# zhao-zilong/Fed-TGAN

Measured on AMD Instinct MI355X. Metric: sec_per_epoch, lower is better.
Workload: dtype bf16; 1 GPU; model=Fed-TGAN CTGAN (G 256x256 residual+BN, D 256x256 pack10, WGAN-GP slerp), global_batch=500, parallelism=fed1, rows_per_client=40000, n_sample=40000, steps_per_epoch=80, backend=hip, data_plane=none

## Files before the change

### csrc/bindings.cpp

```cpp
#include <ATen/ATen.h>
#include <c10/hip/HIPStream.h>
#include <torch/library.h>

#include <cstring>
#include <utility>
#include <string>
#include <vector>

#include "comm/rccl_comm.h"
#include "host/csv_writer.h"
#include "kernels/launch.h"

using at::Tensor;
using c10::optional;

namespace {

hipStream_t cur_stream() { return c10::hip::getCurrentHIPStream().stream(); }

void check_f32_2d(const Tensor& t, const char* name) {
  TORCH_CHECK(t.is_cuda(), name, " must be a GPU tensor");
  TORCH_CHECK(t.scalar_type() == at::kFloat, name, " must be float32");
  TORCH_CHECK(t.dim() == 2, name, " must be 2-D");
  TORCH_CHECK(t.size(1) <= 1 || t.stride(1) == 1, name, " must have unit column stride");
// ... 2016 lines not shown
bool is_checked() { return true; }
#else
bool is_checked() { return false; }
#endif

std::string py_float(double x) { return fedtgan::format_py_float(x); }

int64_t set_tuning(const std::string& key, int64_t value) {
  if (key == "colown_dbg") {
    TORCH_CHECK(value >= 0 && value <= 7, "colown_dbg: bit mask 0..7");
    const int64_t prev = fedtgan::g_colown_dbg;
    fedtgan::g_colown_dbg = (int)value;
    return prev;
  }
  if (key == "bn_cols") {
    TORCH_CHECK(value == 4 || value == 8 || value == 16, "bn_cols must be 4, 8 or 16");
    const int64_t prev = fedtgan::g_bn_cols;
    fedtgan::g_bn_cols = (int)value;
    return prev;
  }
  if (key == "decode_rows") {
    TORCH_CHECK(value >= 0 && value <= 2, "decode_rows: 0 per cell, 1 per row, 2 per row over Philox quads");
    const int prev = fedtgan::g_decode_rows;
    fedtgan::g_decode_rows = (int)value;
    return prev;
  }
  if (key == "chain_pre") {
    TORCH_CHECK(value >= 0 && value <= 2, "chain_pre: 0, 1 or 2");
    const int prev = fedtgan::g_chain_pre;
    fedtgan::g_chain_pre = (int)value;
    return prev;
  }
  if (key == "chain_rows") {
    TORCH_CHECK(value == 1 || value == 2, "chain_rows: 1 or 2");
    const int prev = fedtgan::g_chain_rows;
    fedtgan::g_chain_rows = (int)value;
    return prev;
  }
  if (key == "chain_coalesced") {
    const int prev = fedtgan::g_chain_coalesced;
    fedtgan::g_chain_coalesced = value ? 1 : 0;
    return prev;
  }
  if (key == "gp_threads") {
    TORCH_CHECK(value == 256 || value == 1024, "gp_threads: 256 or 1024");
    const int prev = fedtgan::g_gp_threads;
    fedtgan::g_gp_threads = (int)value;
    return prev;
  }
  if (key == "bn_threads") {
    TORCH_CHECK(value == 512 || value == 1024, "bn_threads: 512 or 1024");
    const int prev = fedtgan::g_bn_threads;
    fedtgan::g_bn_threads = (int)value;
    return prev;
  }
  if (key == "act_rowreg_narrow") {
    TORCH_CHECK(value >= 0 && value <= 2, "act_rowreg_narrow: 0, 1 or 2");
    const int prev = fedtgan::g_act_rowreg_narrow;
    fedtgan::g_act_rowreg_narrow = (int)value;
    return prev;
  }
  if (key == "gp_split") {
    const int prev = fedtgan::g_gp_split;
    fedtgan::g_gp_split = value ? 1 : 0;
    return prev;
  }
  if (key == "act_row_mode") {
    TORCH_CHECK(value >= 0 && value <= 2, "act_row_mode: 0 per-wave, 1 row (LDS image), 2 row (registers; forward)");
    const int prev = fedtgan::g_act_row_mode;
    fedtgan::g_act_row_mode = (int)value;
    return prev;
  }
  if (key == "xcd_clients") {
    TORCH_CHECK(value == 0 || value == 1, "xcd_clients: 0 or 1");
    const int64_t prev = fedtgan::g_xcd_clients;
    fedtgan::g_xcd_clients = (int)value;
    return prev;
  }
  if (key == "adam_store") {
    TORCH_CHECK(value == 0 || value == 2 || value == 16, "adam_store: 0 plain, 2 nt, 16 sc1");
    const int64_t prev = fedtgan::g_adam_store;
    fedtgan::g_adam_store = (int)value;
    return prev;
  }
  if (key == "adam_u_min") {
    TORCH_CHECK(value >= 0, "adam_u_min: >= 0");
    const int64_t prev = fedtgan::g_adam_u_min;
    fedtgan::g_adam_u_min = value;
    return prev;
  }
  if (key == "bnb_first") {
    const int64_t prev = fedtgan::g_bnb_first;
    fedtgan::g_bnb_first = value ? 1 : 0;
    return prev;
  }
  if (key == "bnb_cols") {
    TORCH_CHECK(value == 4 || value == 8, "bnb_cols: 4 or 8");
    const int64_t prev = fedtgan::g_bnb_cols;
    fedtgan::g_bnb_cols = (int)value;
    return prev;
  }
  if (key == "vgm_split") {
    TORCH_CHECK(value >= 0 && value <= 64, "vgm_split: 0..64");
    const int64_t prev = fedtgan::g_vgm_split;
    fedtgan::g_vgm_split = (int)value;
    return prev;
// ... 329 lines not shown
```

### csrc/kernels/ctgan_ops.hip

```cpp
#include <algorithm>
#include <stdexcept>
#include <string>

#include "common.h"
#include "launch.h"
#include "adam_cs.h"

namespace fedtgan {

int g_xcd_clients = 1;
ClientBatch& client_batch() {
  static thread_local ClientBatch cb{1, 0, 0, nullptr, 0};
  return cb;
}

void check_slab(const void* p, const char* what) {
  const ClientBatch& cb = client_batch();
  if (cb.k <= 1 || p == nullptr) return;
  const char* c = static_cast<const char*>(p);
  if (c < cb.base || c >= cb.base + cb.stride)
    throw std::runtime_error(std::string("batched launch: ") + what +
                             " is not in client 0's arena slab (every buffer of a batched step must be)");
}

// ... 754 lines not shown
#pragma unroll
    for (int u = 0; u < TU; ++u) {
      const int j = min(j0 + u * NTH + tid, sl.cols - 1);
      ra[u] = a[j];
      fb[u] = y[j];
    }
#pragma unroll
    for (int u = 0; u < TU; ++u) {
      const int j = j0 + u * NTH + tid;
      if (j < sl.cols) o[j] = wa * ra[u] + wb * fb[u];
    }
  }
}

template <int NW, bool BT_ = false>
__global__ __launch_bounds__(NW * 64) void activate_rowblk_kernel(const float* __restrict__ logits, int ldl,
                                                                  float* __restrict__ out, int ldo, int rows,
                                                                  SpanTables sp, float inv_tau, uint64_t seed,
                                                                  const uint64_t* ctr, uint32_t stream_id,
                                                                  SlerpFuse sl, ClientBatch cb) {
  const BIdx bi_ = batch_bidx<BT_>(cb.xcd);
  extern __shared__ float act_smem[];
  if (bi_.z) {
    const int64_t co = (int64_t)bi_.z * cb.stride;
    logits = cptr(logits, co);
    out = cptr(out, co);
    ctr = cptr(ctr, co);
    client_off(sp, co);
    client_off(sl, co);
    seed += (uint64_t)bi_.z * cb.seed_step;
  }
  constexpr int NTH = NW * 64;
  const int tid = threadIdx.x, lane = tid & 63, wv = tid >> 6;
  const int r = bi_.x;
  const int D = sp.dim, S = sp.n_span;
  const float* x = logits + (size_t)r * ldl;
  const int* einfo = sp.packed;
  const int* kind = einfo + D;
  const int* start = kind + S;
  const int* width = start + S;
  float* vs = act_smem;
  float* smax = vs + D;
  float* ssum = smax + S;
  float* red = ssum + S;
  float* y = out + (size_t)r * ldo;
  const bool do_sl = sl.real != nullptr && r < sl.rows;
  const float* a = do_sl ? sl.real + (size_t)r * sl.ld : x;
  const int j = wv * 64 + lane;
  const bool in = j < D;
  const int jc = min(j, D - 1);
  float xv = x[jc];
  const int ic = einfo[jc];
  const float ar = a[jc];
  const uint64_t step = ctr ? *ctr : 0ull;
  if (in) {
    RngArgs rng{seed, ctr, stream_id};
    const uint4 u4 = rng4(rng, step, ((uint64_t)r << 20) + (uint64_t)(wv >> 2) * 64u + (uint64_t)lane);
    const int q = wv & 3;
    const uint32_t u = q == 0 ? u4.x : q == 1 ? u4.y : q == 2 ? u4.z : u4.w;
    if (!(ic & EI_SOFTMAX)) {
      xv = tanhf(xv);
      y[j] = xv;
    } else {
      xv = (xv + gumbel(u)) * inv_tau;
      vs[j] = xv;
    }
  }
  __syncthreads();
  for (int s2 = tid; s2 < S; s2 += NTH) {
    if (kind[s2] == 0) continue;
    const int st = start[s2], w = width[s2];
    const float* v = vs + st;
    float m = -INFINITY;
    int i = 0;
    for (; i + 4 <= w; i += 4) m = fmaxf(fmaxf(m, fmaxf(v[i], v[i + 1])), fmaxf(v[i + 2], v[i + 3]));
    for (; i < w; ++i) m = fmaxf(m, v[i]);
    float e0 = 0.f, e1 = 0.f;
    i = 0;
    for (; i + 2 <= w; i += 2) {
      e0 += __expf(v[i] - m);
      e1 += __expf(v[i + 1] - m);
    }
    if (i < w) e0 += __expf(v[i] - m);
    smax[s2] = m;
    ssum[s2] = 1.f / (e0 + e1);
  }
  __syncthreads();
  if (in && (ic & EI_SOFTMAX)) {
    const int s2 = ic & (EI_SOFTMAX - 1);
    xv = __expf(xv - smax[s2]) * ssum[s2];
    y[j] = xv;
  }
  if (!do_sl) return;
  float saa = 0.f, sbb = 0.f, sab = 0.f;
  if (in) {
    saa = ar * ar;
    sbb = xv * xv;
    sab = ar * xv;
  }
  constexpr int TU = 2;
  float ra[TU], fb[TU];
#pragma unroll
  for (int u = 0; u < TU; ++u) {
    const int jt = min(D + u * NTH + tid, sl.cols - 1);
    ra[u] = a[jt];
    fb[u] = y[jt];
  }
#pragma unroll
  for (int u = 0; u < TU; ++u)
    if (D + u * NTH + tid < sl.cols) {
      saa += ra[u] * ra[u];
      sbb += fb[u] * fb[u];
      sab += ra[u] * fb[u];
    }
  for (int jt = D + TU * NTH + tid; jt < sl.cols; jt += NTH) {
    const float ra2 = a[jt], fb2 = y[jt];
    saa += ra2 * ra2;
    sbb += fb2 * fb2;
    sab += ra2 * fb2;
  }
  const float3 tot = block_sum3<NW>(saa, sbb, sab, red);
  RngArgs srng{seed, ctr, sl.stream};
  const float alpha = u01(rng4(srng, step, (uint64_t)r).x);
  float wa, wb;
  slerp_weights(tot.x, tot.y, tot.z, alpha, wa, wb);
  float* o = sl.out + (size_t)r * sl.ld;
  if (in) o[j] = wa * ar + wb * xv;
#pragma unroll
  for (int u = 0; u < TU; ++u) {
    const int jt = D + u * NTH + tid;
    if (jt < sl.cols) o[jt] = wa * ra[u] + wb * fb[u];
  }
  for (int jt = D + TU * NTH + tid; jt < sl.cols; jt += NTH) o[jt] = wa * a[jt] + wb * y[jt];
}

template <bool BT_ = false>
__global__ __launch_bounds__(ROW_WAVES * 64) void act_bwd_ce_row_kernel(const float* __restrict__ dact, int ldd,
                                                                        const float* __restrict__ act, int lda,
                                                                        const float* __restrict__ logits, int ldl,
                                                                        SpanTables sp, const int* __restrict__ col,
                                                                        const int* __restrict__ opt,
                                                                        float* __restrict__ dl, int ldg, int rows,
                                                                        float inv_tau, float* loss, int loss_per_row,
                                                                        ClientBatch cb) {
  const BIdx bi_ = batch_bidx<BT_>(cb.xcd);
  extern __shared__ float act_smem[];
  if (bi_.z) {
    const int64_t co = (int64_t)bi_.z * cb.stride;
    dact = cptr(dact, co);
    act = cptr(act, co);
    logits = cptr(logits, co);
    col = cptr(col, co);
    opt = cptr(opt, co);
    dl = cptr(dl, co);
    loss = cptr(loss, co);
    client_off(sp, co);
  }
  const int tid = threadIdx.x, lane = tid & 63, wv = tid >> 6;
  const int r = bi_.x;
  const int D = sp.dim, S = sp.n_span;
  const float* g = dact + (size_t)r * ldd;
  const float* y = act + (size_t)r * lda;
  const float* x = logits + (size_t)r * ldl;
  const int cr = col[r];
  const int orow = opt[r];
  const ActSmem t = act_stage_tables(sp, act_smem);
  float* xs = t.rows;
  float* stat = xs + D;
  int* cspan = reinterpret_cast<int*>(stat + S);
  float* lse_sh = stat + S + 1;
  float* d = dl + (size_t)r * ldg;
  for (int s2 = tid; s2 < S; s2 += blockDim.x) stat[s2] = 0.f;
  if (tid == 0) *cspan = -1;
  __syncthreads();
  for (int s2 = tid; s2 < S; s2 += blockDim.x)
    if (t.kind[s2] != 0 && t.cidx[s2] == cr) *cspan = s2;
// ... 837 lines not shown
  const float* uw = jb.dot_w ? jb.dot_w : jb.w;
  float s = 0.f, s2 = 0.f;
#pragma unroll 8
  for (int r = grp; r < jb.rows; r += CS_GROUPS) {
    const float a = jb.a[(size_t)r * jb.lda + cc];
    s += (jb.w ? jb.w[r] : 1.f) * a;
    if (jb.dot_w) s2 += jb.dot_w[r] * a;
  }
  part[0][grp][threadIdx.x % CS_COLS] = s;
  part[1][grp][threadIdx.x % CS_COLS] = s2;
  __syncthreads();
  if (grp == 0) {
    float t = 0.f, t2 = 0.f;
    for (int i = 0; i < CS_GROUPS; ++i) {
      t += part[0][i][threadIdx.x];
      t2 += part[1][i][threadIdx.x];
    }
    if (c < jb.cols && jb.out) jb.out[c] = t;
    if (jb.dot_v) {
      float d = c < jb.cols ? (jb.dot_w ? t2 : t) * jb.dot_v[c] : 0.f;
      if (bi_.x == 0 && jb.dot_e) {
        float ws = 0.f;
        for (int r = threadIdx.x; r < jb.rows; r += 64) ws += uw ? uw[r] : 1.f;
        d += wave_sum(ws) * (threadIdx.x == 0 ? jb.dot_e[0] : 0.f);
      }
      d = wave_sum(d);
      if (threadIdx.x == 0) atomicAdd(jb.dot_out, d);
    }
  }
}

void launch_colsum(const ColsumJob* jobs, int n_jobs, hipStream_t stream) {
  ColsumBatch bt{};
  int maxc = 0;
  n_jobs = std::min(n_jobs, 8);
  for (int i = 0; i < n_jobs; ++i) {
    bt.jobs[i] = jobs[i];
    maxc = std::max(maxc, jobs[i].cols);
  }
  bt.n_jobs = n_jobs;
  if (n_jobs == 0 || maxc == 0) return;
  const ClientBatch cb = client_batch();
  if (cb.k > 1)
    for (int i = 0; i < n_jobs; ++i)
      check_slabs("colsum job", bt.jobs[i].a, bt.jobs[i].out, bt.jobs[i].w, bt.jobs[i].dot_v, bt.jobs[i].dot_e,
                  bt.jobs[i].dot_out, bt.jobs[i].dot_w);
  hipLaunchKernelGGL((client_batch().xcd ? colsum_kernel<true> : colsum_kernel<false>), dim3((maxc + CS_COLS - 1) / CS_COLS, n_jobs, cb.k), dim3(CS_COLS * CS_GROUPS), 0,
                     stream, bt, cb);
}

constexpr int BN_THREADS = 512, BN_WAVES = BN_THREADS / 64;
int g_bn_cols = 8;
int g_bn_threads = 512;
static int bn_cols_for_launch() { return g_bn_cols; }

constexpr int BN_MAXG = 2;

template <int COLS, int NV, int NTH = BN_THREADS>
__device__ __forceinline__ void bn_colsum(float (&v)[NV], float* sh) {
  constexpr int NWV = NTH / 64;
  const int lane = threadIdx.x & 63, wv = threadIdx.x >> 6, lc = threadIdx.x % COLS;
#pragma unroll
  for (int k = 0; k < NV; ++k) {
#pragma unroll
    for (int o = COLS; o < 64; o <<= 1) v[k] += __shfl_xor(v[k], o, 64);
    if (lane < COLS) sh[(k * NWV + wv) * COLS + lc] = v[k];
  }
  __syncthreads();
#pragma unroll
  for (int k = 0; k < NV; ++k) {
    float t = 0.f;
#pragma unroll
    for (int w = 0; w < NWV; ++w) t += sh[(k * NWV + w) * COLS + lc];
    v[k] = t;
  }
  __syncthreads();
}

struct BnStat {
  float mu, var, is;
};

__device__ __forceinline__ void bn_loads_issued() { __builtin_amdgcn_sched_barrier(0); }

__device__ __forceinline__ float bn_sq(float d) {
#pragma clang fp contract(off)
  return d * d;
}

__device__ __forceinline__ void bn_acc(float& s, float& s2, float d) {
  s += d;
  s2 += bn_sq(d);
}

__device__ __forceinline__ BnStat bn_stat(float s, float s2, float shift, int rpg, float eps) {
#pragma clang fp contract(off)
  BnStat st;
  const float m = s / (float)rpg;
  st.mu = shift + m;
  st.var = fmaxf(__builtin_fmaf(-m, m, s2 / (float)rpg), 0.f);
  st.is = rsqrtf(st.var + eps);
  return st;
}

__device__ __forceinline__ void bn_ema(float& m, float& v, const BnStat& st, float momentum, float unb) {
#pragma clang fp contract(off)
// ... 27 lines not shown
    beta = cptr(beta, co);
    out = cptr(out, co);
    nhat = cptr(nhat, co);
    mean = cptr(mean, co);
    invstd = cptr(invstd, co);
    rm = cptr(rm, co);
    rv = cptr(rv, co);
  }

  constexpr int GROUPS = NTH / COLS;
  __shared__ float sh[2 * BN_MAXG * (NTH / 64) * COLS];
  const int lc = threadIdx.x % COLS, grp = threadIdx.x / COLS;
  const int c = bi_.x * COLS + lc;
  const bool ok = c < cols;
  const int cc = min(c, cols - 1);
  const int rpg = rows / groups;
  const float sh0 = a[cc], sh1 = a[(size_t)min(rpg, rows - 1) * lda + cc];
  const float gm = gamma[cc], bt = beta[cc], rm0 = rm[cc], rv0 = rv[cc];
  float x[MAXR];
  float s[2 * BN_MAXG] = {0.f, 0.f, 0.f, 0.f};
#pragma unroll
  for (int i = 0; i < MAXR; ++i) x[i] = a[(size_t)min(grp + i * GROUPS, rows - 1) * lda + cc];
  bn_loads_issued();
#pragma unroll
  for (int i = 0; i < MAXR; ++i) {
    const int r = grp + i * GROUPS;
    const bool g1 = r >= rpg;
    const float dv = x[i] - (g1 ? sh1 : sh0);
    const float d = (r < rows) ? dv : 0.f;
    if (g1) bn_acc(s[1], s[3], d); else bn_acc(s[0], s[2], d);
  }
  bn_colsum<COLS, 2 * BN_MAXG, NTH>(s, sh);
  const BnStat st0 = bn_stat(s[0], s[2], sh0, rpg, eps), st1 = bn_stat(s[1], s[3], sh1, rpg, eps);
  if (grp == 0 && ok) {
    const float unb = bn_unbias(rpg);
    float m = rm0, v = rv0;
    mean[c] = st0.mu;
    invstd[c] = st0.is;
    bn_ema(m, v, st0, momentum, unb);
    if (groups > 1) {
      mean[(size_t)cols + c] = st1.mu;
      invstd[(size_t)cols + c] = st1.is;
      bn_ema(m, v, st1, momentum, unb);
    }
    rm[c] = m;
    rv[c] = v;
  }
  if (!ok) return;
#pragma unroll
  for (int i = 0; i < MAXR; ++i) {
    const int r = grp + i * GROUPS;
    if (r < rows) {
      const float n = bn_nhat(x[i], r >= rpg ? st1 : st0);
      nhat[(size_t)r * ldn + c] = n;
      out[(size_t)r * ldo + c] = bn_affine_relu(n, gm, bt);
    }
  }
}

template <int COLS, bool BT_ = false>
__global__ __launch_bounds__(BN_THREADS) void bn_relu_train_stream_kernel(
    const float* __restrict__ a, int lda, const float* __restrict__ gamma, const float* __restrict__ beta,
    float* __restrict__ out, int ldo, float* __restrict__ nhat, int ldn, float* __restrict__ mean,
    float* __restrict__ invstd, float* __restrict__ rm, float* __restrict__ rv, int rows, int cols, int groups,
    float momentum, float eps, ClientBatch cb) {
  const BIdx bi_ = batch_bidx<BT_>(cb.xcd);
  if (bi_.z) {
    const int64_t co = (int64_t)bi_.z * cb.stride;
    a = cptr(a, co);
    gamma = cptr(gamma, co);
    beta = cptr(beta, co);
    out = cptr(out, co);
    nhat = cptr(nhat, co);
    mean = cptr(mean, co);
    invstd = cptr(invstd, co);
    rm = cptr(rm, co);
    rv = cptr(rv, co);
  }

  constexpr int GROUPS = BN_THREADS / COLS;
  __shared__ float sh[2 * BN_MAXG * BN_WAVES * COLS];
  const int lc = threadIdx.x % COLS, grp = threadIdx.x / COLS;
  const int c = bi_.x * COLS + lc;
  const bool ok = c < cols;
  const int cc = min(c, cols - 1);
  const int rpg = rows / groups;
  const float sh0 = a[cc], sh1 = a[(size_t)min(rpg, rows - 1) * lda + cc];
  float s[2 * BN_MAXG] = {0.f, 0.f, 0.f, 0.f};
  for (int r = grp; r < rows; r += GROUPS) {
    const float v = a[(size_t)r * lda + cc];
    const bool g1 = r >= rpg;
    const float d = v - (g1 ? sh1 : sh0);
    if (g1) { s[1] += d; s[3] += d * d; } else { s[0] += d; s[2] += d * d; }
  }
  bn_colsum<COLS, 2 * BN_MAXG>(s, sh);
  const float m0 = s[0] / (float)rpg, m1 = s[1] / (float)rpg;
  const float mu0 = sh0 + m0, mu1 = sh1 + m1;
  const float var0 = fmaxf(s[2] / (float)rpg - m0 * m0, 0.f);
  const float var1 = fmaxf(s[3] / (float)rpg - m1 * m1, 0.f);
  const float is0 = rsqrtf(var0 + eps), is1 = rsqrtf(var1 + eps);
  if (grp == 0 && ok) {
    const float unb = (float)rpg / (float)max(rpg - 1, 1);
    float m = rm[c], v = rv[c];
    mean[c] = mu0;
    invstd[c] = is0;
    m = (1.f - momentum) * m + momentum * mu0;
// ... 91 lines not shown
    }
  __syncthreads();
  if (bi_.y == 0 && t < BNA_COLS && c0 + t < cols) {
    const int c = c0 + t;
    const float unb = (float)rpg / (float)max(rpg - 1, 1);
    float m = rm[c], v = rv[c];
    for (int b = 0; b < groups; ++b) {
      mean[(size_t)b * cols + c] = st[t][b][0];
      invstd[(size_t)b * cols + c] = st[t][b][1];
      m = (1.f - momentum) * m + momentum * st[t][b][0];
      v = (1.f - momentum) * v + momentum * st[t][b][2] * unb;
    }
    rm[c] = m;
    rv[c] = v;
  }
  if (r >= rows) return;
  const int bb = (groups > 1 && r >= rpg) ? 1 : 0;
#pragma unroll
  for (int e = 0; e < 4; ++e) {
    const int cl = cq + e, c = c0 + cl;
    if (c >= cols) break;
    const float nv = (x[e] - st[cl][bb][0]) * st[cl][bb][1];
    nhat[(size_t)r * ldn + c] = nv;
    const float y = nv * gamma[c] + beta[c];
    out[(size_t)r * ldo + c] = y > 0.f ? y : 0.f;
  }
}

void launch_bn_relu_apply(const float* a, int lda, const float* part, int n_tiles, const float* gamma,
                          const float* beta, float* out, int ldo, float* nhat, int ldn, float* mean, float* invstd,
                          float* rm, float* rv, int rows, int cols, int groups, float momentum, float eps,
                          hipStream_t stream) {
  const ClientBatch cb = client_batch();
  if (cb.k > 1) check_slabs("bn_relu_apply operand", a, part, gamma, beta, out, nhat, mean, invstd, rm, rv);
  const dim3 grid((cols + BNA_COLS - 1) / BNA_COLS, (rows + BNA_ROWS - 1) / BNA_ROWS, cb.k);
  hipLaunchKernelGGL((client_batch().xcd ? bn_relu_apply_kernel<true> : bn_relu_apply_kernel<false>), grid, dim3(BNA_THREADS), 0, stream, a, lda, part, n_tiles, gamma, beta,
                     out, ldo, nhat, ldn, mean, invstd, rm, rv, rows, cols, groups, momentum, eps, cb);
}

template <int COLS>
static void bn_train_cols(const float* a, int lda, const float* gamma, const float* beta, float* out, int ldo,
                          float* nhat, int ldn, float* mean, float* invstd, float* rm, float* rv, int rows, int cols,
                          int groups, float momentum, float eps, hipStream_t stream) {
  constexpr int GROUPS = BN_THREADS / COLS;
  const ClientBatch cb = client_batch();
  if (cb.k > 1) check_slabs("bn_relu_train operand", a, gamma, beta, out, nhat, mean, invstd, rm, rv);
  const dim3 grid((cols + COLS - 1) / COLS, 1, cb.k), block(BN_THREADS);
  if (g_bn_threads == 1024 && rows <= 8 * (1024 / COLS)) {
    hipLaunchKernelGGL((client_batch().xcd ? bn_relu_train_kernel<COLS, 8, true, 1024> : bn_relu_train_kernel<COLS, 8, false, 1024>),
                       grid, dim3(1024), 0, stream, a, lda, gamma, beta, out, ldo, nhat, ldn, mean, invstd, rm, rv, rows,
                       cols, groups, momentum, eps, cb);
    return;
  }
#define BN_TRAIN_LAUNCH(R)                                                                                          \
  hipLaunchKernelGGL((client_batch().xcd ? bn_relu_train_kernel<COLS, R, true> : bn_relu_train_kernel<COLS, R, false>), grid, block, 0, stream, a, lda, gamma, beta, out, ldo, nhat, \
                     ldn, mean, invstd, rm, rv, rows, cols, groups, momentum, eps, cb)
  if (rows <= 4 * GROUPS) BN_TRAIN_LAUNCH(4);
  else if (rows <= 8 * GROUPS) BN_TRAIN_LAUNCH(8);
  else if (rows <= 16 * GROUPS) BN_TRAIN_LAUNCH(16);
  else if (rows <= 32 * GROUPS) BN_TRAIN_LAUNCH(32);
  else if (rows <= 64 * GROUPS) BN_TRAIN_LAUNCH(64);
  else
    hipLaunchKernelGGL((client_batch().xcd ? bn_relu_train_stream_kernel<COLS, true> : bn_relu_train_stream_kernel<COLS, false>), grid, block, 0, stream, a, lda, gamma, beta, out, ldo,
                       nhat, ldn, mean, invstd, rm, rv, rows, cols, groups, momentum, eps, cb);
#undef BN_TRAIN_LAUNCH
}

void launch_bn_relu_train(const float* a, int lda, const float* gamma, const float* beta, float* out, int ldo,
                          float* nhat, int ldn, float* mean, float* invstd, float* rm, float* rv, int rows, int cols,
                          int groups, float momentum, float eps, hipStream_t stream) {
  const int bc = bn_cols_for_launch();
  if (bc == 4)
    bn_train_cols<4>(a, lda, gamma, beta, out, ldo, nhat, ldn, mean, invstd, rm, rv, rows, cols, groups, momentum, eps,
                     stream);
  else if (bc == 16)
    bn_train_cols<16>(a, lda, gamma, beta, out, ldo, nhat, ldn, mean, invstd, rm, rv, rows, cols, groups, momentum,
                      eps, stream);
  else
    bn_train_cols<8>(a, lda, gamma, beta, out, ldo, nhat, ldn, mean, invstd, rm, rv, rows, cols, groups, momentum, eps,
                     stream);
}

template <int COLS, int MAXR, bool BT_ = false, int NTH = BN_THREADS>
__global__ __launch_bounds__(NTH) void bn_relu_bwd_kernel(
    const float* __restrict__ dr, int lddr, const float* __restrict__ r_, int ldr, const float* __restrict__ nhat,
    int ldn, const float* __restrict__ gamma, const float* __restrict__ invstd, float* __restrict__ da, int ldda,
    float* __restrict__ dgamma, float* __restrict__ dbeta, float* __restrict__ dbias, int rows, int cols, ClientBatch cb) {
  const BIdx bi_ = batch_bidx<BT_>(cb.xcd);
  if (bi_.z) {
    const int64_t co = (int64_t)bi_.z * cb.stride;
    dr = cptr(dr, co);
    r_ = cptr(r_, co);
    nhat = cptr(nhat, co);
    gamma = cptr(gamma, co);
    invstd = cptr(invstd, co);
    da = cptr(da, co);
    dgamma = cptr(dgamma, co);
    dbeta = cptr(dbeta, co);
    dbias = cptr(dbias, co);
  }

  constexpr int GROUPS = NTH / COLS;
  __shared__ float sh[3 * (NTH / 64) * COLS];
  const int lc = threadIdx.x % COLS, grp = threadIdx.x / COLS;
  const int c = bi_.x * COLS + lc;
  const bool ok = c < cols;
  const int cc = min(c, cols - 1);
// ... 480 lines not shown
```

### csrc/kernels/gemm.hip

```cpp
#include <algorithm>
#include <type_traits>

#include "common.h"
#include "launch.h"
#include "adam_cs.h"
#include "bn_bwd.h"

namespace fedtgan {

#if FT_CHECKED
__device__ unsigned g_check_gemm = 0u;
unsigned check_status_gemm() {
  unsigned v = 0u, z = 0u;
  (void)hipMemcpyFromSymbol(&v, HIP_SYMBOL(g_check_gemm), sizeof(v));
  (void)hipMemcpyToSymbol(HIP_SYMBOL(g_check_gemm), &z, sizeof(z));
  return v;
}
#else
unsigned check_status_gemm() { return 0u; }
#endif

typedef __attribute__((ext_vector_type(8))) short bf16x8;
typedef __attribute__((ext_vector_type(4))) float f32x4;
typedef __attribute__((ext_vector_type(4))) unsigned u32x4;
// ... 912 lines not shown
#pragma unroll
  for (int z = 0; z < SMAX; ++z) part[z] = g.ws[(size_t)min(z, splits - 1) * total + idx];
  float acc[4] = {0.f, 0.f, 0.f, 0.f};
#pragma unroll
  for (int z = 0; z < SMAX; ++z)
    if (z < splits) acc[z & 3] += part[z];
  float v = g.alpha * ((acc[0] + acc[1]) + (acc[2] + acc[3]));
  float* cp = g.c + (size_t)m * g.ldc + n;
  if (g.beta != 0.f) v += g.beta * (*cp);
  if (g.bias) v += g.bias[n];
  if (g.oh_w) v += onehot_term(g, m, n);
  if constexpr (MASK) return v * g.ms[(size_t)m * g.ldms + n];
  return apply_epi(g, v, m, n, step, idx);
}

template <int SMAX, bool BT_ = false>
__global__ __launch_bounds__(256) void gemm_splitk_epilogue(GemmArgs g) {
  const BIdx bi_ = batch_bidx<BT_>(g.xcd_cl);
  if (bi_.z) client_view(g, bi_.z);
  const size_t total = (size_t)g.M * g.N;
  const uint64_t step = (g.epi == EPI_LRELU_DROPOUT && g.rng_ctr) ? *g.rng_ctr : 0ull;
  for (size_t idx = (size_t)bi_.x * blockDim.x + threadIdx.x; idx < total; idx += (size_t)gridDim.x * blockDim.x) {
    const int m = (int)(idx / g.N), n = (int)(idx % g.N);
    st_out(g.c, (size_t)m * g.ldc + n, splitk_value<SMAX>(g, idx, m, n, step), g.wt);
  }
}

constexpr int CH_MAXK = 1024, CH_COLS = 64;
int g_chain_coalesced = 0;
int g_chain_pre = 1;
int g_chain_rows = 2;
template <int SMAX, bool MASK = false, bool BT_ = false, bool PRE = false, int ROWS = 1, bool ACH = false>
__global__ __launch_bounds__(256) void chain_epilogue_kernel(GemmArgs g, GemmArgs t) {
  static_assert(ROWS == 1 || PRE, "two rows per workgroup only with the prefetched tail");
  static_assert(!ACH || (!MASK && !BT_), "the fused A-chain takes the D-head chain of one client");
  const BIdx bi_ = batch_bidx<BT_>(g.xcd_cl);
  __shared__ __attribute__((aligned(16))) float row[ROWS][CH_MAXK];
  __shared__ float part[ROWS][4][CH_COLS];
  if (bi_.z) {
    client_view(g, bi_.z);
    client_view(t, bi_.z);
  }
  const int m0 = bi_.x * ROWS, s = bi_.y;
  const uint64_t step = (g.epi == EPI_LRELU_DROPOUT && g.rng_ctr) ? *g.rng_ctr : 0ull;
  constexpr int PQ = 16;
  const bool pre = PRE && !t.chain_co && g.N == 16 * PQ;
  float4 wp[PRE ? PQ : 1];
  if (pre) {
    const int jp = min(s * CH_COLS + (int)(threadIdx.x & (CH_COLS - 1)), t.N - 1);
    const float4* w4 = reinterpret_cast<const float4*>(t.b + (size_t)jp * t.ldb) + (threadIdx.x >> 6) * PQ;
#pragma unroll
    for (int k = 0; k < (PRE ? PQ : 1); ++k) wp[k] = w4[k];
  }
  for (int n = threadIdx.x; n < g.N; n += blockDim.x) {
#pragma unroll
    for (int r = 0; r < ROWS; ++r) {
      const int m = m0 + r;
      float v = 0.f;
      if (ROWS == 1 || m < g.M) {
        if constexpr (SMAX > 0) {
          v = splitk_value<SMAX, MASK>(g, (size_t)m * g.N + n, m, n, step);
          if (s == 0) st_out(g.c, (size_t)m * g.ldc + n, v, g.wt);
        } else {
          v = g.c[(size_t)m * g.ldc + n];
        }
      }
      row[r][n] = v;
    }
  }
  __syncthreads();
  const int jl = threadIdx.x & (CH_COLS - 1), kq = threadIdx.x >> 6;
  const int j = s * CH_COLS + jl;
  if (!PRE && !ACH && t.chain_co) {
    constexpr int JW = CH_COLS / 4;
    const int lane = threadIdx.x & 63, m = m0;
    float p[JW];
#pragma unroll
    for (int jj = 0; jj < JW; ++jj) p[jj] = 0.f;
    for (int k0 = 0; k0 < g.N; k0 += 256) {
      const int k = k0 + 4 * lane;
      const bool kin = k < g.N;
      const float4 x = kin ? *reinterpret_cast<const float4*>(row[0] + k) : make_float4(0.f, 0.f, 0.f, 0.f);
      float4 w[JW];
#pragma unroll
      for (int jj = 0; jj < JW; ++jj) {
        const int jc = min(s * CH_COLS + kq * JW + jj, t.N - 1);
        w[jj] = *reinterpret_cast<const float4*>(t.b + (size_t)jc * t.ldb + min(k, g.N - 4));
      }
#pragma unroll
      for (int jj = 0; jj < JW; ++jj)
        if (kin) p[jj] += (w[jj].x * x.x + w[jj].y * x.y) + (w[jj].z * x.z + w[jj].w * x.w);
    }
#pragma unroll
    for (int jj = 0; jj < JW; ++jj) {
      const float tsum = wave_sum(p[jj]);
      if (lane == 0) part[0][0][kq * JW + jj] = tsum;
    }
    __syncthreads();
    if (kq == 0 && j < t.N) {
      float v = t.alpha * part[0][0][jl];
      if (t.bias) v += t.bias[j];
      const uint64_t st = (t.epi == EPI_LRELU_DROPOUT && t.rng_ctr) ? *t.rng_ctr : 0ull;
      if constexpr (MASK) t.c[(size_t)m * t.ldc + j] = v * t.ms[(size_t)m * t.ldms + j];
      else t.c[(size_t)m * t.ldc + j] = apply_epi(t, v, m, j, st, (uint64_t)m * t.N + j);
    }
    return;
  }
  const int q4 = g.N / 16;
  if (pre) {
#pragma unroll
    for (int r = 0; r < ROWS; ++r) {
      const float4* r4 = reinterpret_cast<const float4*>(row[r]) + kq * PQ;
      float a0 = 0.f, a1 = 0.f;
#pragma unroll
      for (int k = 0; k < (PRE ? PQ : 1); ++k) {
        const float4 w = wp[k], x = r4[k];
        a0 = fmaf(w.x, x.x, a0);
        a1 = fmaf(w.y, x.y, a1);
        a0 = fmaf(w.z, x.z, a0);
        a1 = fmaf(w.w, x.w, a1);
      }
      part[r][kq][jl] = a0 + a1;
    }
  } else {
    float a0 = 0.f, a1 = 0.f;
    if (j < t.N) {
      const float4* w4 = reinterpret_cast<const float4*>(t.b + (size_t)j * t.ldb) + kq * q4;
      const float4* r4 = reinterpret_cast<const float4*>(row[0]) + kq * q4;
#pragma unroll 4
      for (int k = 0; k < q4; ++k) {
        const float4 w = w4[k], x = r4[k];
        a0 = fmaf(w.x, x.x, a0);
        a1 = fmaf(w.y, x.y, a1);
        a0 = fmaf(w.z, x.z, a0);
        a1 = fmaf(w.w, x.w, a1);
      }
    }
    part[0][kq][jl] = a0 + a1;
  }
  __syncthreads();
  if (kq == 0 && j < t.N) {
    const uint64_t st = (t.epi == EPI_LRELU_DROPOUT && t.rng_ctr) ? *t.rng_ctr : 0ull;
#pragma unroll
    for (int r = 0; r < ROWS; ++r) {
      const int m = m0 + r;
      if (ROWS > 1 && m >= g.M) break;
      float v = t.alpha * ((part[r][0][jl] + part[r][1][jl]) + (part[r][2][jl] + part[r][3][jl]));
      if (t.bias) v += t.bias[j];
      if constexpr (MASK) t.c[(size_t)m * t.ldc + j] = v * t.ms[(size_t)m * t.ldms + j];
      else t.c[(size_t)m * t.ldc + j] = apply_epi(t, v, m, j, st, (uint64_t)m * t.N + j);
    }
  }
  if constexpr (ACH) {
    __shared__ float a1s[ROWS][CH_COLS];
    __shared__ unsigned ach_last;
    if (kq == 0) {
#pragma unroll
      for (int r = 0; r < ROWS; ++r) {
        const int m = m0 + r;
        a1s[r][jl] = (j < t.N && (ROWS == 1 || m < g.M)) ? t.head_a[(size_t)m * t.ldha + j] : 0.f;
      }
    }
    __syncthreads();
    const int jn = min(CH_COLS, t.N - s * CH_COLS);
    for (int i = threadIdx.x; i < g.N; i += blockDim.x) {
      float acc[ROWS];
#pragma unroll
      for (int r = 0; r < ROWS; ++r) acc[r] = 0.f;
      const float* wc = t.b + (size_t)s * CH_COLS * t.ldb + i;
      for (int c = 0; c < jn; ++c) {
        const float w = wc[(size_t)c * t.ldb];
#pragma unroll
        for (int r = 0; r < ROWS; ++r) acc[r] = fmaf(a1s[r][c], w, acc[r]);
      }
#pragma unroll
      for (int r = 0; r < ROWS; ++r) {
        const int m = m0 + r;
        if (ROWS == 1 || m < g.M)
          __hip_atomic_store(&t.ach_ws[((size_t)s * g.M + m) * g.N + i], acc[r], __ATOMIC_RELAXED,
                             __HIP_MEMORY_SCOPE_AGENT);
      }
    }
    asm volatile("s_waitcnt vmcnt(0)" ::: "memory");
    __syncthreads();
    if (threadIdx.x == 0) {
      const unsigned tk = __hip_atomic_fetch_add(&t.ach_cnt[bi_.x], 1u, __ATOMIC_RELAXED, __HIP_MEMORY_SCOPE_AGENT);
      const unsigned last = tk == gridDim.y - 1 ? 1u : 0u;
      if (last) __hip_atomic_store(&t.ach_cnt[bi_.x], 0u, __ATOMIC_RELAXED, __HIP_MEMORY_SCOPE_AGENT);
      ach_last = last;
    }
    __syncthreads();
    if (ach_last == 0u) return;
    for (int i = threadIdx.x; i < g.N; i += blockDim.x) {
#pragma unroll
      for (int r = 0; r < ROWS; ++r) {
        const int m = m0 + r;
        if (ROWS > 1 && m >= g.M) break;
        float sum = 0.f;
        for (int q = 0; q < (int)gridDim.y; ++q)
          sum += __hip_atomic_load(&t.ach_ws[((size_t)q * g.M + m) * g.N + i], __ATOMIC_RELAXED,
// ... 648 lines not shown
```

### csrc/kernels/launch.h

```cpp
#pragma once
#include <hip/hip_runtime.h>
#include <stdint.h>

namespace fedtgan {

enum Epilogue : int { EPI_NONE = 0, EPI_LRELU_DROPOUT = 1, EPI_MASK = 2, EPI_RELU = 3, EPI_BN_EVAL_RELU = 4 };

struct RngArgs;

struct ClientBatch {
  int k;
  int64_t stride;
  uint64_t seed_step;
  const char* base;
  int xcd;
};
extern int g_xcd_clients;
ClientBatch& client_batch();
void check_slab(const void* p, const char* what);
void require_unbatched(const char* what);
template <class... P>
inline void check_slabs(const char* what, P... ps) {
  (check_slab((const void*)ps, what), ...);
}
// ... 92 lines not shown
  int n_real;
  float* step_bump;
  float* step_bump2;
  float* metrics;
  int zero_metrics;
  uint64_t seed;
  const uint64_t* rng_ctr;
  uint32_t rng_stream;
  int draws;
  int64_t draw_h, draw_x, draw_col;
  ClientBatch cb;
};

void launch_sample(const SampleArgs& a, hipStream_t stream);

struct SpanTables {
  const int* start;
  const int* width;
  const int* kind;
  const int* cond_idx;
  const int* packed;
  int n_span;
  int dim;
};
inline int span_packed_len(int dim, int n_span) { return (dim + 4 * n_span + 3) & ~3; }

size_t activation_smem_bytes(const SpanTables& sp);

struct SlerpFuse {
  const float* real;
  float* out;
  int ld, cols;
  int rows;
  uint32_t stream;
};
void launch_activate(const float* logits, int ldl, float* out, int ldo, int rows, SpanTables sp, float tau,
                     uint64_t seed, const uint64_t* ctr, uint32_t stream_id, SlerpFuse sl, hipStream_t stream);

void launch_act_bwd_ce(const float* dact, int ldd, const float* act, int lda, const float* logits, int ldl, SpanTables sp,
                       const int* col, const int* opt, float* dlogits, int ldg, int rows, float tau, float* loss,
                       int loss_per_row, hipStream_t stream);

void launch_slerp(const float* real, const float* fake, float* out, int rows, int cols, int ld, uint64_t seed,
                  const uint64_t* ctr, uint32_t stream_id, hipStream_t stream);

void launch_gp_scale(const float* g, int ldg, float* out, int ldo, int rows, int cols, float lam, float* loss,
                     int loss_per_row, float* ws, int64_t ws_n, hipStream_t stream);
extern int g_gp_split;
extern int g_chain_coalesced;
extern int g_chain_pre;
extern int g_chain_rows;
extern int g_gp_threads;
extern int g_bn_threads;
extern int g_act_rowreg_narrow;

struct OnehotWJob {
  const float* dy;
  float* w;
  int ldy, ldw, n;
};
struct OnehotWBatch {
  OnehotWJob jobs[4];
  int n_jobs, B;
  const int* col;
  const int* opt;
  const int* cond_off;
};
void launch_onehot_wgrad(const OnehotWBatch& bt, int zero, hipStream_t stream);

void launch_d_head(const float* d, int ldd, const float* ms, int ldms, const float* v, const float* e,
                   const float* coef, const float* wloss, float* y, float* a, int lda, int rows, int cols, float* loss,
                   hipStream_t stream);

struct ColsumJob {
  const float* a;
  int lda, rows, cols;
  float* out;
  const float* w;
  const float* dot_v;
  const float* dot_e;
  float* dot_out;
  const float* dot_w;
};
void launch_colsum(const ColsumJob* jobs, int n_jobs, hipStream_t stream);

constexpr int ACS_COLS = 16, ACS_GROUPS = 64;
struct AdamColsum {
  ColsumJob jobs[8];
  int n_jobs;
  int vec[8];
  int blk_start[9];
  int64_t own_lo[8], own_hi[8];
  int dot_self[8];
  int64_t skip_lo, skip_hi;
  int64_t skip2_lo, skip2_hi;
};
bool launch_gemm_shortk_adam(GemmArgs g, hipStream_t stream);
void launch_adam_colsum(float* p, const float* g, float* m, float* v, const float* step, int64_t n, float lr, float b1,
                        float b2, float eps, float wd, uint64_t* rng_ctr_bump, const AdamColsum& cs,
                        hipStream_t stream);
bool launch_gemm_adam(GemmArgs g, float* p, const float* gr, float* m, float* v, const float* step, int64_t n,
                      float lr, float b1, float b2, float eps, float wd, uint64_t* rng_ctr_bump, const AdamColsum& cs,
                      hipStream_t stream);

extern int g_gemm_xcd_remap;
extern int g_gemm_xcd_nmajor;
// ... 553 lines not shown
```

Before: 0.01509 s/epoch.

## Split BN train across row-slice blocks, hoist slerp/epilogue loads earlier

```diff
diff --git a/csrc/bindings.cpp b/csrc/bindings.cpp
--- a/csrc/bindings.cpp
+++ b/csrc/bindings.cpp
@@ -2092,6 +2092,12 @@
     TORCH_CHECK(value == 512 || value == 1024, "bn_threads: 512 or 1024");
     const int prev = fedtgan::g_bn_threads;
     fedtgan::g_bn_threads = (int)value;
+    return prev;
+  }
+  if (key == "bn_slices") {
+    TORCH_CHECK(value == 1 || value == 2 || value == 4, "bn_slices: 1, 2 or 4");
+    const int prev = fedtgan::g_bn_slices;
+    fedtgan::g_bn_slices = (int)value;
     return prev;
   }
   if (key == "act_rowreg_narrow") {
diff --git a/csrc/kernels/ctgan_ops.hip b/csrc/kernels/ctgan_ops.hip
--- a/csrc/kernels/ctgan_ops.hip
+++ b/csrc/kernels/ctgan_ops.hip
@@ -830,7 +830,20 @@
   float xv = x[jc];
   const int ic = einfo[jc];
   const float ar = a[jc];
+  constexpr int TU = 2;
+  float ra[TU], fb[TU];
+#pragma unroll
+  for (int u = 0; u < TU; ++u) {
+    const int jt = do_sl ? min(D + u * NTH + tid, sl.cols - 1) : jc;
+    ra[u] = a[jt];
+    fb[u] = y[jt];
+  }
   const uint64_t step = ctr ? *ctr : 0ull;
+  float alpha = 0.f;
+  if (do_sl) {
+    RngArgs srng{seed, ctr, sl.stream};
+    alpha = u01(rng4(srng, step, (uint64_t)r).x);
+  }
   if (in) {
     RngArgs rng{seed, ctr, stream_id};
     const uint4 u4 = rng4(rng, step, ((uint64_t)r << 20) + (uint64_t)(wv >> 2) * 64u + (uint64_t)lane);
@@ -876,14 +889,6 @@
     sbb = xv * xv;
     sab = ar * xv;
   }
-  constexpr int TU = 2;
-  float ra[TU], fb[TU];
-#pragma unroll
-  for (int u = 0; u < TU; ++u) {
-    const int jt = min(D + u * NTH + tid, sl.cols - 1);
-    ra[u] = a[jt];
-    fb[u] = y[jt];
-  }
 #pragma unroll
   for (int u = 0; u < TU; ++u)
     if (D + u * NTH + tid < sl.cols) {
@@ -898,8 +903,6 @@
     sab += ra2 * fb2;
   }
   const float3 tot = block_sum3<NW>(saa, sbb, sab, red);
-  RngArgs srng{seed, ctr, sl.stream};
-  const float alpha = u01(rng4(srng, step, (uint64_t)r).x);
   float wa, wb;
   slerp_weights(tot.x, tot.y, tot.z, alpha, wa, wb);
   float* o = sl.out + (size_t)r * sl.ld;
@@ -1843,6 +1846,7 @@
 constexpr int BN_THREADS = 512, BN_WAVES = BN_THREADS / 64;
 int g_bn_cols = 8;
 int g_bn_threads = 512;
+int g_bn_slices = 2;
 static int bn_cols_for_launch() { return g_bn_cols; }
 
 constexpr int BN_MAXG = 2;
@@ -1976,6 +1980,82 @@
     const int r = grp + i * GROUPS;
     if (r < rows) {
       const float n = bn_nhat(x[i], r >= rpg ? st1 : st0);
+      nhat[(size_t)r * ldn + c] = n;
+      out[(size_t)r * ldo + c] = bn_affine_relu(n, gm, bt);
+    }
+  }
+}
+
+template <int COLS, int MAXR>
+__global__ __launch_bounds__(BN_THREADS) void bn_relu_train_sliced_kernel(
+    const float* __restrict__ a, int lda, const float* __restrict__ gamma, const float* __restrict__ beta,
+    float* __restrict__ out, int ldo, float* __restrict__ nhat, int ldn, float* __restrict__ mean,
+    float* __restrict__ invstd, float* __restrict__ rm, float* __restrict__ rv, int rows, int cols, int slices,
+    float momentum, float eps) {
+  constexpr int GROUPS = BN_THREADS / COLS, NB = MAXR / 2 + 1;
+  __shared__ float sh[2 * BN_MAXG * BN_WAVES * COLS];
+  const int lc = threadIdx.x % COLS, grp = threadIdx.x / COLS;
+  const int c = blockIdx.x * COLS + lc;
+  const bool ok = c < cols;
+  const int cc = min(c, cols - 1);
+  const int rpg = rows / 2;
+  if (blockIdx.y == 0) {
+    const float sh0 = a[cc], sh1 = a[(size_t)rpg * lda + cc];
+    const float rm0 = rm[cc], rv0 = rv[cc];
+    float x[MAXR];
+    float s[2 * BN_MAXG] = {0.f, 0.f, 0.f, 0.f};
+#pragma unroll
+    for (int i = 0; i < MAXR; ++i) x[i] = a[(size_t)min(grp + i * GROUPS, rows - 1) * lda + cc];
+    bn_loads_issued();
+#pragma unroll
+    for (int i = 0; i < MAXR; ++i) {
+      const int r = grp + i * GROUPS;
+      const bool g1 = r >= rpg;
+      const float dv = x[i] - (g1 ? sh1 : sh0);
+      const float d = (r < rows) ? dv : 0.f;
+      if (g1) bn_acc(s[1], s[3], d); else bn_acc(s[0], s[2], d);
+    }
+    bn_colsum<COLS, 2 * BN_MAXG>(s, sh);
+    if (grp != 0 || !ok) return;
+    const BnStat st0 = bn_stat(s[0], s[2], sh0, rpg, eps), st1 = bn_stat(s[1], s[3], sh1, rpg, eps);
+    const float unb = bn_unbias(rpg);
+    float m = rm0, v = rv0;
+    mean[c] = st0.mu;
+    invstd[c] = st0.is;
+    bn_ema(m, v, st0, momentum, unb);
+    mean[(size_t)cols + c] = st1.mu;
+    invstd[(size_t)cols + c] = st1.is;
+    bn_ema(m, v, st1, momentum, unb);
+    rm[c] = m;
+    rv[c] = v;
+    return;
+  }
+  const int role = (int)blockIdx.y - 1, b = role / slices, sl = role - b * slices;
+  const int lo = b * rpg, hi = lo + rpg;
+  const int i0 = lo / GROUPS;
+  const float shift = a[(size_t)lo * lda + cc];
+  const float gm = gamma[cc], bt = beta[cc];
+  float x[NB];
+  float s[2] = {0.f, 0.f};
+#pragma unroll
+  for (int j = 0; j < NB; ++j) x[j] = a[(size_t)min(grp + (i0 + j) * GROUPS, rows - 1) * lda + cc];
+  bn_loads_issued();
+#pragma unroll
+  for (int j = 0; j < NB; ++j) {
+    const int r = grp + (i0 + j) * GROUPS;
+    const float dv = x[j] - shift;
+    const float d = (r >= lo && r < hi) ? dv : 0.f;
+    bn_acc(s[0], s[1], d);
+  }
+  bn_colsum<COLS, 2>(s, sh);
+  const BnStat st = bn_stat(s[0], s[1], shift, rpg, eps);
+  if (!ok) return;
+  const int jlo = sl * NB / slices, jhi = (sl + 1) * NB / slices;
+#pragma unroll
+  for (int j = 0; j < NB; ++j) {
+    const int r = grp + (i0 + j) * GROUPS;
+    if (j >= jlo && j < jhi && r >= lo && r < hi) {
+      const float n = bn_nhat(x[j], st);
       nhat[(size_t)r * ldn + c] = n;
       out[(size_t)r * ldo + c] = bn_affine_relu(n, gm, bt);
     }
@@ -2173,7 +2253,21 @@
                        cols, groups, momentum, eps, cb);
     return;
   }
-#define BN_TRAIN_LAUNCH(R)                                                                                          \
+  const auto apart = [&](const float* p, int ld) {
+    return p + (size_t)rows * ld <= a || a + (size_t)rows * lda <= p;
+  };
+  if (g_bn_slices > 1 && g_bn_threads == 512 && groups == 2 && cb.k == 1 && rows <= 16 * GROUPS && apart(out, ldo) && apart(nhat, ldn)) {
+    const dim3 sgrid(grid.x, 1 + 2 * g_bn_slices);
+#define BN_SLICED_LAUNCH(R)                                                                                         \
+  hipLaunchKernelGGL((bn_relu_train_sliced_kernel<COLS, R>), sgrid, block, 0, stream, a, lda, gamma, beta, out, ldo, \
+                     nhat, ldn, mean, invstd, rm, rv, rows, cols, g_bn_slices, momentum, eps)
+    if (rows <= 4 * GROUPS) BN_SLICED_LAUNCH(4);
+    else if (rows <= 8 * GROUPS) BN_SLICED_LAUNCH(8);
+    else BN_SLICED_LAUNCH(16);
+#undef BN_SLICED_LAUNCH
+    return;
+  }
+#define BN_TRAIN_LAUNCH(R)                                                                                        \
   hipLaunchKernelGGL((client_batch().xcd ? bn_relu_train_kernel<COLS, R, true> : bn_relu_train_kernel<COLS, R, false>), grid, block, 0, stream, a, lda, gamma, beta, out, ldo, nhat, \
                      ldn, mean, invstd, rm, rv, rows, cols, groups, momentum, eps, cb)
   if (rows <= 4 * GROUPS) BN_TRAIN_LAUNCH(4);
diff --git a/csrc/kernels/gemm.hip b/csrc/kernels/gemm.hip
--- a/csrc/kernels/gemm.hip
+++ b/csrc/kernels/gemm.hip
@@ -988,6 +988,27 @@
 #pragma unroll
     for (int k = 0; k < (PRE ? PQ : 1); ++k) wp[k] = w4[k];
   }
+  float e_bias = 0.f, e_hv = 0.f, e_ms[ROWS], e_hc[ROWS];
+  uint64_t e_st = 0ull;
+  if constexpr (PRE) {
+#pragma unroll
+    for (int r = 0; r < ROWS; ++r) e_ms[r] = e_hc[r] = 0.f;
+    if ((threadIdx.x >> 6) == 0) {
+      const int jp = min(s * CH_COLS + (int)threadIdx.x, t.N - 1);
+      if (t.bias) e_bias = t.bias[jp];
+      if constexpr (MASK) {
+#pragma unroll
+        for (int r = 0; r < ROWS; ++r) e_ms[r] = t.ms[(size_t)min(m0 + r, g.M - 1) * t.ldms + jp];
+      } else {
+        if (t.epi == EPI_LRELU_DROPOUT && t.rng_ctr) e_st = *t.rng_ctr;
+        if (t.epi == EPI_LRELU_DROPOUT && t.head_a) {
+          e_hv = t.head_v[jp];
+#pragma unroll
+          for (int r = 0; r < ROWS; ++r) e_hc[r] = t.head_coef[min(m0 + r, g.M - 1)];
+        }
+      }
+    }
+  }
   for (int n = threadIdx.x; n < g.N; n += blockDim.x) {
 #pragma unroll
     for (int r = 0; r < ROWS; ++r) {
@@ -1082,6 +1103,24 @@
       const int m = m0 + r;
       if (ROWS > 1 && m >= g.M) break;
       float v = t.alpha * ((part[r][0][jl] + part[r][1][jl]) + (part[r][2][jl] + part[r][3][jl]));
+      if constexpr (PRE) {
+        if (t.bias) v += e_bias;
+        if constexpr (MASK) {
+          t.c[(size_t)m * t.ldc + j] = v * e_ms[r];
+        } else if (t.epi == EPI_LRELU_DROPOUT) {
+          const float sl = v > 0.f ? 1.f : t.slope;
+          RngArgs rng{t.seed, t.rng_ctr, t.rng_stream};
+          const uint4 rr = rng4(rng, e_st, (uint64_t)m * t.N + j);
+          const float keep = (u01(rr.x) >= t.p_drop) ? 1.f / (1.f - t.p_drop) : 0.f;
+          const float f = sl * keep;
+          t.ms[(size_t)m * t.ldms + j] = f;
+          if (t.head_a) t.head_a[(size_t)m * t.ldha + j] = e_hc[r] * e_hv * f;
+          t.c[(size_t)m * t.ldc + j] = v * f;
+        } else {
+          t.c[(size_t)m * t.ldc + j] = apply_epi(t, v, m, j, e_st, (uint64_t)m * t.N + j);
+        }
+        continue;
+      }
       if (t.bias) v += t.bias[j];
       if constexpr (MASK) t.c[(size_t)m * t.ldc + j] = v * t.ms[(size_t)m * t.ldms + j];
       else t.c[(size_t)m * t.ldc + j] = apply_epi(t, v, m, j, st, (uint64_t)m * t.N + j);
diff --git a/csrc/kernels/launch.h b/csrc/kernels/launch.h
--- a/csrc/kernels/launch.h
+++ b/csrc/kernels/launch.h
@@ -168,6 +168,7 @@
 extern int g_chain_rows;
 extern int g_gp_threads;
 extern int g_bn_threads;
+extern int g_bn_slices;
 extern int g_act_rowreg_narrow;
 
 struct OnehotWJob {
```

New measurement: 0.01475 s/epoch, median of 6. -2.2%, faster.
